# bbbranjan/scConsensus

Measured on AMD Instinct MI355X. Metric: end-to-end DE+distance cell-pairs/sec at config B (26k PBMC shape), higher is better.
Workload: dtype f64

## Files before the change

scconsensus_amd/csrc/scc_de.cpp:

```cpp
#include "scc_internal.hpp"

#include <array>
#include <cstring>
#include <memory>
#include <thread>

using namespace scc_rt;

enum { DE_FULL = 0, DE_SHARD = 1, DE_FINISH = 2, DE_SHARD_REC = 3, DE_FINISH_REC = 4 };

extern "C" {
int scc_rec_blocks(long long cells);
hipError_t scc_launch_rec_count(const uint8_t* flags, int G, int P, int glo, int ghi, int all, uint32_t* cnt,
                                hipStream_t st);
hipError_t scc_launch_rec_pack(const uint8_t* flags, int G, int P, int glo, int ghi, int all, const long long* off,
                               const double* p, const double* lfc, const double* pct1, const double* pct2,
                               const long long* u2, const long long* t, scc_de_record* out, hipStream_t st);
hipError_t scc_launch_rec_scatter(const scc_de_record* rec, long long n, int G, int P, double* p, double* lfc,
                                  double* pct1, double* pct2, long long* u2, long long* t, uint8_t* flags, int* err,
                                  int plo, int phi, hipStream_t st);
}

struct RecIO {
    void* out = nullptr;
// ... 9 lines not shown

extern "C" void scc_rank_split_diag(hipStream_t st, int ngenes);

enum IngestRoute {
    INGEST_NONE = 0,
    INGEST_FULL = 1,
    INGEST_LEAN = 2,
    INGEST_MIRROR = 3,
};

struct DePlan {
    const scc_dataset* ds;
    const scc_de_params* prm;
    void* shard;
    const RecIO* rio;
    int stage;
    bool shard_stage, finish_stage;
    bool pairs_only;
    int G, N, K, P, glo, ghi;
    int64_t GK, nnz1;
    size_t PG;
    bool fast, norank, all_pairs;
    bool markers;
    int test;
    std::vector<int> nclu;
    int nkept, nc, nc_kept, ns, gt, ntile, nwaves;
    size_t o_ccp0, o_cccode, o_sccc0, o_clcc, o_nclu, o_code8, tab_n;
    int ntp_max, cap_s, cap_m, wave_target, bucket_cap, item_cap, bucket_target;
    size_t acc_n;
    bool resplit, stamps;
    int fat_cap;
    IngestRoute route;
    bool try_mirror;
    double log_thr;
};

struct DeBuffers {
    int *d_tab, *d_nodg, *d_splitg, *d_counts, *d_err, *d_tested, *d_union, *d_nu, *d_genebk;
    const int *d_perm, *d_ccp0, *d_cccode, *d_sccc0, *d_clcc, *d_nclu;
    const signed char* d_code8;
    uint32_t *d_cnt, *d_cntpos, *d_cntneg, *d_gix, *d_gwin, *d_cscr;
    long long *d_gstart, *d_scan, *d_rowoff, *d_bnd;
    unsigned long long *d_keys, *d_keys2, *d_acc, *d_gkmin, *d_first;
    unsigned long long *accS, *accE, *accX, *accF;
    uint8_t *d_gcode, *d_gsc, *d_codes2, *d_flags;
    ScRankItem *d_items, *d_sbk;
    unsigned int* d_hbg;
    dd *d_wexp, *d_gexp;
    dd* d_sume;
    double *d_mx, *d_me, *d_vx, *d_mpos, *d_m2pos, *d_minpos, *d_maxpos;
    double *d_p, *d_lfc, *d_pct1, *d_pct2;
    long long *d_u2, *d_t;
    uint32_t* gene_tp;
    int* gene_nt;
    char* tp_scr;
    ScRankItem *fatbk, *fat2;
    int4 *rsseg, *fatg;
    unsigned long long* st_buf;
    uint32_t* d_rc;
    long long *d_roff, *d_rscr;
    int* d_row_gene;
    double *d_row_p, *d_row_q, *d_row_lfc, *d_row_pct1, *d_row_pct2;
    long long *d_row_u2, *d_row_t;
    uint8_t* d_row_flags;
    double* d_slow_q;
    uint8_t* d_slow_de;
// ... 399 lines not shown
    if (!ds->m_gptr) return SCC_OK;
    pl->route = INGEST_MIRROR;
    if (int rc = ensure_vorder(c, pl, B)) return rc;
    if (ds->d_tbnd) {
        hipFree(ds->d_tbnd);
        ds->d_tbnd = nullptr;
    }
    return SCC_OK;
}

static long long* gene_starts(const DePlan& pl, const DeBuffers& B)
{
    const bool whole = pl.glo == 0 && pl.ghi == pl.G;
    return pl.route == INGEST_MIRROR && whole && pl.nkept == pl.N ? pl.ds->m_gptr : B.d_gstart;
}

static int ingest_mirror(scc_ctx* c, const DePlan& pl, const DeBuffers& B)
{
    const scc_dataset* ds = pl.ds;
    const int G = pl.G, N = pl.N, K = pl.K, glo = pl.glo, ghi = pl.ghi, nc = pl.nc;
    hipStream_t s0 = c->s0;
    Scope sc(c, "ingest", s0);
    HIPCHK(c, scc_launch_de_clear(B.d_err, B.d_counts, pl.norank ? nullptr : B.d_acc, (long long)pl.acc_n, B.d_first,
                                  (int)G, glo, ghi, s0));
    HIPCHK(c, hipMemcpyAsync(B.d_nodg, ds->d_nodg, sizeof(int) * N, hipMemcpyDeviceToDevice, s0));
    const bool whole = glo == 0 && ghi == G;
    long long* gstart_run = gene_starts(pl, B);
    if (gstart_run == B.d_gstart) {
        uint32_t* d_total = B.d_cnt + (size_t)nc * G;
        if (!whole) HIPCHK(c, hipMemsetAsync(d_total, 0, sizeof(uint32_t) * G, s0));
        HIPCHK(c, scc_launch_mirror_total(ds->m_gptr, ds->m_cell, B.d_code8, glo, ghi, d_total, s0));
        HIPCHK(c, scc_launch_scan(d_total, G, B.d_gstart, B.d_scan, B.d_gstart + G, s0));
    }
    HIPCHK(c, scc_launch_mirror_regroup(ds->m_gptr, ds->m_cell, ds->m_key, B.d_code8, whole ? ds->m_order : nullptr,
                                        glo, ghi, K, G, B.d_clcc, gstart_run, B.d_cnt, B.d_keys, s0));
    return SCC_OK;
}

static int ingest_transpose(scc_ctx* c, const DePlan& pl, const DeBuffers& B)
{
    const scc_dataset* ds = pl.ds;
    const int G = pl.G, N = pl.N, glo = pl.glo, ghi = pl.ghi, nc = pl.nc, ntile = pl.ntile;
    const bool fast = pl.fast, lean = pl.route == INGEST_LEAN;
    const bool hist_rng = lean && (glo > 0 || ghi < G);
    const bool hist_ro = lean && !hist_rng;
    hipStream_t s0 = c->s0;
    Scope sc(c, "ingest", s0);
    HIPCHK(c, scc_launch_de_clear(B.d_err, B.d_counts, pl.norank ? nullptr : B.d_acc, (long long)pl.acc_n, B.d_first,
                                  (int)G, glo, ghi, s0));
    if (lean && !ds->d_tbnd) {
        const size_t tb_bytes = sizeof(long long) * (size_t)N * (ntile + 1);
        size_t mfree = 0, mtot = 0;
        const bool room = hipMemGetInfo(&mfree, &mtot) == hipSuccess && tb_bytes <= mfree / 4;
        (void)hipGetLastError();
        if (!room || hipMalloc((void**)&ds->d_tbnd, tb_bytes) != hipSuccess) {
            (void)hipGetLastError();
            ds->d_tbnd = nullptr;
        } else {
            HIPCHK(c, scc_launch_tile_bounds(ds->d_indptr, ds->d_rows, N, pl.gt, ntile, ds->d_tbnd, s0));
        }
    }
    const long long* tbnd = lean ? ds->d_tbnd : nullptr;
    if ((hist_ro || (hist_rng && ds->no_zeros)) && tbnd && env_int("SCC_COUNT_RO", 1) != 0)
        HIPCHK(c, scc_launch_ingest_count_ro(ds->d_indptr, ds->d_rows, G, B.d_perm, B.d_ccp0, B.d_cccode, nc,
                                             hist_rng ? glo : 0, hist_rng ? ghi : G, tbnd, B.d_cnt, s0));
    else
        HIPCHK(c, scc_launch_ingest_hist(ds->d_indptr, ds->d_rows, ds->d_vals, ds->d_dense, G, B.d_perm, B.d_ccp0,
                                         B.d_cccode, nc, ntile, B.d_cnt, B.d_bnd, B.d_nodg, B.d_wexp, fast ? 0 : 1, glo,
                                         ghi, hist_rng ? 1 : (hist_ro ? 2 : 0), tbnd, B.d_err, s0));
    if (lean) HIPCHK(c, hipMemcpyAsync(B.d_nodg, ds->d_nodg, sizeof(int) * N, hipMemcpyDeviceToDevice, s0));
    int cg0 = 0, cg1 = G;
    if (hist_rng) {
        scc_ingest_count_range(G, glo, ghi, &cg0, &cg1);
        HIPCHK(c, hipMemsetAsync(B.d_cnt + (size_t)nc * G, 0, sizeof(uint32_t) * G, s0));
    }
    HIPCHK(c, scc_launch_ingest_colscan(B.d_cnt, nc, pl.nc_kept, G, cg0, cg1, B.d_cscr, s0));
    const uint32_t* d_total = B.d_cnt + (size_t)nc * G;
    HIPCHK(c, scc_launch_scan(d_total, G, B.d_gstart, B.d_scan, B.d_gstart + G, s0));
    HIPCHK(c, scc_launch_ingest_scatter(ds->d_indptr, ds->d_rows, ds->d_vals, ds->d_dense, G, B.d_perm, B.d_ccp0,
                                        B.d_sccc0, pl.ns, B.d_cnt, B.d_gstart, B.d_bnd, tbnd, ntile, glo, ghi, B.d_keys,
                                        s0));
    if (!fast) HIPCHK(c, scc_launch_reduce_dd(B.d_wexp, pl.nwaves, B.d_gexp, s0));
    return SCC_OK;
}

static int gene_stats(scc_ctx* c, const DePlan& pl, const DeBuffers& B)
{
    Scope sc(c, "gene_stats", c->s0);
    ScStatsLaunch S{};
    S.gstart = gene_starts(pl, B);
    S.keys = B.d_keys;
    S.G = pl.G, S.K = pl.K, S.glo = pl.glo, S.gn = pl.ghi - pl.glo;
    S.mode = pl.prm->mode, S.test = pl.test;
    S.n_clu = B.d_nclu, S.coff = B.d_cnt, S.cl_cc = B.d_clcc;
    S.mean_x = B.d_mx, S.mean_e = B.d_me, S.cnt_pos = B.d_cntpos, S.cnt_neg = B.d_cntneg;
    S.var_x = B.d_vx;
    S.mean_pos = B.d_mpos, S.m2_pos = B.d_m2pos, S.min_pos = B.d_minpos, S.max_pos = B.d_maxpos;
    S.sum_e = B.d_sume;
    HIPCHK(c, scc_launch_gene_stats(&S, c->s0));
    return SCC_OK;
}

static int slow_threshold(scc_ctx* c, const DePlan& pl, const DeBuffers& B, double* log_thr)
{
    double gx[2];
    HIPCHK(c, hipMemcpyAsync(gx, B.d_gexp, sizeof(double) * 2, hipMemcpyDeviceToHost, c->s0));
    HIPCHK(c, hipStreamSynchronize(c->s0));
    const double tot = (double)pl.G * (double)pl.N;
    double q = gx[0] / tot;
    double r = std::fma(-q, tot, gx[0]) + gx[1];
    const double mean = q + r / tot;
    *log_thr = std::log(pl.prm->mean_scaling_factor * mean);
    return SCC_OK;
}

static ScTestLaunch test_launch(const scc_ctx* c, const DePlan& pl, const DeBuffers& B)
{
    ScTestLaunch T{};
    T.K = pl.K, T.G = pl.G, T.P = pl.P, T.glo = pl.glo, T.ghi = pl.ghi;
    T.mode = pl.prm->mode, T.test = pl.test, T.all_pairs = pl.all_pairs ? 1 : 0;
    T.min_pct = pl.prm->min_per_cent, T.lfc_thr = pl.prm->log_fc_thrs, T.log_thr = pl.log_thr;
// ... 24 lines not shown
    L.rw_mfma16 = env_int("SCC_RANK_MFMA16", -1);
    L.cross_wave = env_int("SCC_CROSS_WAVE", 0);
    L.bucket_cap = pl.bucket_cap, L.sbuckets = B.d_sbk, L.hbg = B.d_hbg;
    L.gene_bk = B.d_genebk, L.gkmin = B.d_gkmin;
    L.ntp_max = pl.ntp_max, L.item_cap = pl.item_cap, L.items = B.d_items;
    L.counts = B.d_counts, L.split_genes = B.d_splitg;
    L.keys2 = B.d_keys2, L.codes2 = B.d_codes2;
    L.gix = B.d_gix, L.gwin = B.d_gwin, L.gcode = B.d_gcode, L.gsc = B.d_gsc;
    L.nnz = pl.nnz1;
    L.accS = B.accS, L.accE = B.accE, L.accX = B.accX, L.accF = B.accF;
    L.gene_tp = B.gene_tp, L.gene_nt = B.gene_nt;
    if (scc_rank_tables_global(pl.ntp_max, K)) {
        L.tp_global = 1;
        L.tp_scr_stride = scc_rank_tables_stride(pl.ntp_max, K);
        L.tp_scr = B.tp_scr;
    }
    if (pl.resplit) {
        L.fat_cap = L.fat2_cap = pl.fat_cap;
        L.fatbk = B.fatbk, L.rsseg = B.rsseg, L.fatg = B.fatg, L.fat2 = B.fat2;
    }
    return L;
}

static int rank_log(scc_ctx* c, hipStream_t s0, const int* d_counts);

static bool rank_vorder_route(const scc_ctx* c, const DePlan& pl)
{
    const scc_dataset* ds = pl.ds;
    return ds->m_vcell && ds->m_vbk && ds->m_gptr && pl.route == INGEST_MIRROR && pl.fast && !pl.norank &&
           !pl.markers && !pl.shard_stage && pl.glo == 0 && pl.ghi == pl.G && c->peers.empty() &&
           ds->m_vnbk <= pl.bucket_cap && !pl.stamps && env_int("SCC_RANK_VORDER", 1) != 0;
}

static int rank_stage_vorder(scc_ctx* c, const DePlan& pl, const DeBuffers& B, ScRankLaunch& L)
{
    int rc;
    hipStream_t s0 = c->s0;
    const scc_dataset* ds = pl.ds;
    L.vcell = ds->m_vcell, L.vbk_ptr = ds->m_vbk_ptr, L.vbk = ds->m_vbk, L.vgptr = ds->m_gptr;
    L.code8 = B.d_code8;
    L.fatbk = nullptr;
    const int ncu = c->n_cu > 0 ? c->n_cu : 256;
    HIPCHK(c, scc_launch_rank_classify(&L, s0));
    HIPCHK(c, scc_launch_rank_vorder_list(&L, std::max(1, std::min((pl.G + 7) / 8, 1 << 20)), s0));
    if (L.dbg == 7) scc_rank_mfma_stamps(s0, 0);
    const int rw_side = (pl.K > 16 && env_int("SCC_RW_STREAMS", 1) != 0 && L.dbg != 7) ? 2 : 0;
    HIPCHK(c, scc_launch_rank_waves(&L, 8 * ncu, s0, c->sw, rw_side, c->ev_wfork, c->ev_wj));
    if (L.dbg == 7) scc_rank_mfma_stamps(s0, 1);
    HIPCHK(c, scc_launch_rank_cross(&L, 4 * ncu, s0));
    if (env_int("SCC_RANK_LOG", 0) && (rc = rank_log(c, s0, B.d_counts))) return rc;
    g_rank_last_route = 2;
    return SCC_OK;
}

static hipError_t read_counts(const int* d_counts, hipStream_t s0, int* h)
{
    int t[SCC_NCOUNTS * SCC_CNT_STRIDE];
    hipError_t e = hipMemcpyAsync(t, d_counts, sizeof(t), hipMemcpyDeviceToHost, s0);
    if (e == hipSuccess) e = hipStreamSynchronize(s0);
    for (int i = 0; i < SCC_NCOUNTS; ++i) h[i] = t[i * SCC_CNT_STRIDE];
    return e;
}

static int rank_stamps_begin(scc_ctx* c, hipStream_t s0, unsigned long long* st_buf, int item_cap, ScRankLaunch& L)
{
    HIPCHK(c, hipMemsetAsync(st_buf, 0, sizeof(unsigned long long) * 3 * item_cap * 8, s0));
// ... 40 lines not shown
}

static int rank_stamps_report(scc_ctx* c, hipStream_t s0, const unsigned long long* st_buf, int item_cap,
                              const int* d_counts)
{
    std::vector<unsigned long long> h((size_t)3 * item_cap * 8);
    int cnts[SCC_NCOUNTS];
    HIPCHK(c, hipMemcpyAsync(h.data(), st_buf, h.size() * 8, hipMemcpyDeviceToHost, s0));
    HIPCHK(c, read_counts(d_counts, s0, cnts));
    const char* ph[] = {"setup", "sort", "fixup+codes", "partition", "pairs", "ties"};
    fprintf(stderr, "[scc stamps] split genes %d\n", cnts[3]);
    for (int cls = 0; cls < 3; ++cls) {
        double acc[6] = {0, 0, 0, 0, 0, 0};
        int nb = 0;
        for (int b = 0; b < cnts[cls]; ++b) {
            const unsigned long long* t = &h[((size_t)cls * item_cap + b) * 8];
            if (!t[0] || !t[6]) continue;
            for (int q = 0; q < 6; ++q) acc[q] += (double)(t[q + 1] - t[q]);
            ++nb;
        }
        fprintf(stderr, "[scc stamps] rank class %d: %d items (%d full), mean cycles:", cls, cnts[cls], nb);
        for (int q = 0; q < 6; ++q) fprintf(stderr, " %s %.0f", ph[q], nb ? acc[q] / nb : 0.0);
        fprintf(stderr, "\n");
    }
    return SCC_OK;
}

static int rank_stage(scc_ctx* c, const DePlan& pl, const DeBuffers& B)
{
    int rc;
    hipStream_t s0 = c->s0, s1 = c->s1;
    Scope sc(c, "gene_rank", s0);
    ScRankLaunch L = rank_launch(pl, B);
    if (rank_vorder_route(c, pl)) return rank_stage_vorder(c, pl, B, L);
    if (pl.stamps && (rc = rank_stamps_begin(c, s0, B.st_buf, pl.item_cap, L))) return rc;
    HIPCHK(c, scc_launch_rank_classify(&L, s0));
    const int ncu = c->n_cu > 0 ? c->n_cu : 256;
    HIPCHK(c, scc_launch_rank_split(&L, 2 * ncu, s0));
    if (L.dbg >= 9 && (rc = rank_split_clocks(c, s0, B.d_counts))) return rc;
    if (pl.stamps) {
        if ((rc = rank_resplit_clocks(c, s0, L, B.st_buf, pl.item_cap, ncu))) return rc;
    } else {
        const int rw_mode = env_int("SCC_RW_STREAMS", 1);
        const int rs_side = (rw_mode >= 2 || (rw_mode != 0 && pl.ds->nnz > (64ll << 20))) ? 2 : 0;
        HIPCHK(c, scc_launch_rank_resplit(&L, 4 * ncu, s0, c->sw, rs_side, c->ev_wfork, c->ev_wj));
    }
    const bool items_serial = env_int("SCC_ITEMS_SERIAL", 0) != 0;
    hipStream_t si = items_serial ? s0 : s1;
    if (!items_serial) {
        HIPCHK(c, hipEventRecord(c->ev_fork, s0));
        HIPCHK(c, hipStreamWaitEvent(s1, c->ev_fork, 0));
    }
    if (L.dbg == 7) scc_rank_mfma_stamps(s0, 0);
    const int rw_side = (env_int("SCC_RW_STREAMS", 1) != 0 && L.dbg != 7) ? 2 : 0;
    const hipStream_t wsides[2] = {c->sw[0], si};
    HIPCHK(c, scc_launch_rank_waves(&L, 8 * ncu, s0, si != s0 ? wsides : c->sw, rw_side, c->ev_wfork, c->ev_wj));
    if (L.dbg == 7) scc_rank_mfma_stamps(s0, 1);
    HIPCHK(c, scc_launch_rank_items(&L, 1, 2 * ncu, si));
    HIPCHK(c, scc_launch_rank_items(&L, 0, 4 * ncu, si));
    HIPCHK(c, scc_launch_rank_items(&L, 2, ncu, si));
    if (!items_serial) {
        HIPCHK(c, hipEventRecord(c->ev_join, s1));
        HIPCHK(c, hipStreamWaitEvent(s0, c->ev_join, 0));
    }
    HIPCHK(c, scc_launch_rank_cross(&L, 4 * ncu, s0));
    HIPCHK(c, scc_launch_rank_cross_seg(&L, 4 * ncu, s0));
    if (env_int("SCC_RANK_LOG", 0) && (rc = rank_log(c, s0, B.d_counts))) return rc;
// ... 182 lines not shown
        r->n_rows = nrows;
    }
    r->d_nodg = B.d_nodg;
    r->d_row_gene = B.d_row_gene, r->d_row_p = B.d_row_p, r->d_row_q = B.d_row_q, r->d_row_lfc = B.d_row_lfc;
    r->d_row_pct1 = B.d_row_pct1, r->d_row_pct2 = B.d_row_pct2;
    r->d_row_u2 = B.d_row_u2, r->d_row_t = B.d_row_t, r->d_row_flags = B.d_row_flags;
    r->d_p = B.d_p, r->d_q = B.d_slow_q, r->d_lfc = B.d_lfc, r->d_u2 = B.d_u2, r->d_de = B.d_slow_de;
    return r;
}

static int de_run(scc_ctx* c, const scc_dataset* ds, const int32_t* code, int32_t K, const scc_de_params* prm,
                  int stage, int64_t glo64, int64_t ghi64, void* shard, scc_de_result** out,
                  const RecIO* rio = nullptr)
{
    int rc;
    if ((rc = de_check_args(c, ds, code, K, prm, stage, shard, out, rio))) return rc;
    scc_enter(c);
    DePlan pl{};
    if ((rc = de_plan(c, ds, code, K, prm, stage, glo64, ghi64, shard, rio, &pl))) return rc;
    DeBuffers B{};
    if ((rc = de_alloc(c, pl, &B))) return rc;
    if ((rc = ensure_wtab(c, exact_test_max_size(pl.nclu)))) return rc;
    hipStream_t s0 = c->s0;
    c->generation++;
    const int64_t sig[6] = {pl.G, pl.N, K, prm->mode, ds->nnz, (int64_t)(intptr_t)ds};
    if (pl.finish_stage) {
        if (!std::equal(sig, sig + 6, c->shard_sig))
            return fail(c, SCC_ERR_INVALID, "scc_de_finish: this context ran no scc_de_run_shard for these inputs");
        pl.log_thr = c->shard_log_thr;
        if ((rc = stage == DE_FINISH ? finish_load_dense(c, pl, B) : finish_scatter_records(c, pl, B))) return rc;
    } else {
        if ((rc = upload_tables(c, B))) return rc;
        if (pl.try_mirror && (rc = ensure_mirror(c, &pl, B))) return rc;
        g_ingest_last_path = pl.route;
        g_rank_last_route = 1;
        if ((rc = pl.route == INGEST_MIRROR ? ingest_mirror(c, pl, B) : ingest_transpose(c, pl, B))) return rc;
        if ((rc = gene_stats(c, pl, B))) return rc;
        if (!pl.fast && (rc = slow_threshold(c, pl, B, &pl.log_thr))) return rc;
        const ScTestLaunch T = test_launch(c, pl, B);
        {
            Scope sc(c, "pair_filter", s0);
            HIPCHK(c, scc_launch_pair_filter(&T, s0));
        }
        if (!pl.norank && (rc = rank_stage(c, pl, B))) return rc;
        {
            Scope sc(c, "pair_test", s0);
            HIPCHK(c, scc_launch_pair_test(&T, s0));
        }
    }
    if (pl.shard_stage) {
        if ((rc = stage == DE_SHARD ? shard_pack(c, pl, B) : shard_records(c, pl, B))) return rc;
        std::copy(sig, sig + 6, c->shard_sig);
        c->shard_log_thr = pl.log_thr;
        HIPCHK(c, hipStreamSynchronize(s0));
        int e = 0;
        HIPCHK(c, hipMemcpy(&e, B.d_err, sizeof(int), hipMemcpyDeviceToHost));
        if ((rc = de_error(c, e, AT_SHARD))) return rc;
        return note_validated(c, pl, B, e);
    }
    if ((rc = pair_select(c, pl, B)) || pl.pairs_only) return rc;
    if ((rc = stage_pack(c, pl, B))) return rc;
    const int n_union = c->h_stage[0], err_bits = c->h_stage[1];
    if ((rc = de_error(c, err_bits, AT_FULL))) return rc;
    if ((rc = note_validated(c, pl, B, err_bits))) return rc;
    if (n_union < 0 || n_union > pl.G) return fail(c, SCC_ERR_HIP, "union size out of range");
    *out = build_result(c, pl, B, n_union);
    return de_error(c, err_bits, AT_RESULT);
}
// ... 46 lines not shown
    return SCC_OK;
}

extern "C" int scc_de_markers(scc_ctx* c, const scc_dataset* ds, const int32_t* code, int32_t K,
                              const scc_markers_params* mp, scc_de_result** out)
{
    if (!c || !ds || !code || !mp || !out) return fail(c, SCC_ERR_INVALID, "scc_de_markers: null argument");
    *out = nullptr;
    if (ds->ctx != c) return fail(c, SCC_ERR_INVALID, "dataset belongs to another context");
    if (mp->test == SCC_TEST_T || mp->test == SCC_TEST_BIMOD)
        return fail(c, SCC_ERR_UNSUPPORTED, "scc_de_markers: SCC_TEST_WILCOX only");
    if (mp->test != SCC_TEST_WILCOX) return fail(c, SCC_ERR_INVALID, "scc_de_markers: bad test");
    if (K < 2) return fail(c, SCC_ERR_INVALID, "need at least two clusters");
    if (K > kMaxK) return fail(c, SCC_ERR_UNSUPPORTED, "scc_de_markers: K > 128 clusters");
    for (int32_t v : mp->reserved)
        if (v != 0) return fail(c, SCC_ERR_INVALID, "scc_de_markers: reserved fields must be zero");
    scc_de_params dp{};
    dp.mode = SCC_DE_FAST, dp.top_n = mp->top_n, dp.q_val_thrs = mp->q_val_thrs, dp.log_fc_thrs = mp->log_fc_thrs;
    dp.min_per_cent = mp->min_per_cent, dp.fc_thrs = 1.5, dp.mean_scaling_factor = 5.0;
    dp.test_all = mp->test_all ? 1 : 0, dp.test = SCC_TEST_WILCOX;
    int rc;
    scc_enter(c);
    DePlan pl{};
    if ((rc = markers_plan(c, ds, code, K, &dp, &pl))) return rc;
    DeBuffers B{};
    if ((rc = de_alloc(c, pl, &B))) return rc;
    if ((rc = ensure_wtab(c, markers_exact_size(pl.nclu)))) return rc;
    hipStream_t s0 = c->s0;
    c->generation++;
    if ((rc = upload_tables(c, B))) return rc;
    if (pl.try_mirror && (rc = ensure_mirror(c, &pl, B))) return rc;
    g_ingest_last_path = pl.route;
    g_rank_last_route = 1;
    if ((rc = pl.route == INGEST_MIRROR ? ingest_mirror(c, pl, B) : ingest_transpose(c, pl, B))) return rc;
    if ((rc = gene_stats(c, pl, B))) return rc;
    const ScRestTestLaunch T = rest_launch(c, pl, B, mp->only_pos ? 1 : 0);
    {
        Scope sc(c, "rest_filter", s0);
        HIPCHK(c, scc_launch_rest_filter(&T, s0));
    }
    if ((rc = rank_rest_stage(c, pl, B))) return rc;
    {
        Scope sc(c, "rest_test", s0);
        HIPCHK(c, scc_launch_rest_test(&T, s0));
    }
    if ((rc = pair_select(c, pl, B))) return rc;
    if ((rc = stage_pack(c, pl, B))) return rc;
    const int n_union = c->h_stage[0], err_bits = c->h_stage[1];
    if ((rc = de_error(c, err_bits, AT_FULL))) return rc;
    if ((rc = note_validated(c, pl, B, err_bits))) return rc;
    if (n_union < 0 || n_union > pl.G) return fail(c, SCC_ERR_HIP, "union size out of range");
    scc_de_result* r = build_result(c, pl, B, n_union);
    r->d_t = B.d_t;
    *out = r;
    return de_error(c, err_bits, AT_RESULT);
}

static int gene_blocks(scc_ctx* c, const scc_dataset* ds, int D, std::vector<int64_t>& cut)
{
    const int64_t G = ds->G;
    cut.assign(D + 1, 0);
    cut[D] = G;
    if (!ds->dense && ds->gene_w.empty() && ds->nnz > 0) {
        unsigned int* d_h = nullptr;
        int rc = ws(c, "row_hist", (size_t)G, &d_h);
        if (rc) return rc;
// ... 525 lines not shown
```

scconsensus_amd/csrc/scc_ingest.hip:

```cpp
#include "scc_common.hpp"
#include <algorithm>
#include "scc_kernels.hpp"

#define ING_T 256
#define IH_T (64 * SCC_ING_HIST_WAVES)

template <bool DENSE>
__device__ inline void cell_range(const i64* indptr, int c, int G, i64& b, i64& e)
{
    if (DENSE) {
        b = (i64)c * G;
        e = b + G;
    } else {
        b = indptr[c];
        e = indptr[c + 1];
    }
}

__device__ inline i64 wave_lower_bound(const int* __restrict__ rows, i64 lo, i64 hi, int v)
{
    const int lane = threadIdx.x & 63;
    while (hi - lo > 64) {
        const i64 step = (hi - lo + 63) / 64;
        const i64 k = lo + (i64)lane * step;
// ... 913 lines not shown
        }
        __syncthreads();
#pragma unroll
        for (int u = 0; u < MR_PER; ++u)
            if (aa[u] >= 0) {
                const u32 r = (u32)wc16[(wv * MR_PER + u) * SCC_MAX_K + aa[u]] + rk[u];
                const u32 slot = cst[aa[u]] + r;
                if (slot < (u32)MR_CH) {
                    skey[slot] = kk[u];
                    sdst[slot] = dbase[aa[u]] + r;
                }
            }
        __syncthreads();
        const int nk = (int)cst[K];
        for (int i0 = tid; i0 < nk; i0 += 4 * MR_T) {
            u64 kq[4];
            u32 dq[4];
#pragma unroll
            for (int q = 0; q < 4; ++q) {
                const int i = min(i0 + q * MR_T, nk - 1);
                kq[q] = skey[i];
                dq[q] = sdst[i];
            }
#pragma unroll
            for (int q = 0; q < 4; ++q)
                if (i0 + q * MR_T < nk) keys[gs + dq[q]] = kq[q];
        }
        if (c0 + MR_CH >= n) {
            if (tid <= K) cnt[(size_t)cl_cc[tid] * G + g] = coff[tid];
        }
    }
}

__global__ void __launch_bounds__(256) k_mir_segtab(const u32* __restrict__ cnt, int nch, int G, int nseg,
                                                    u32* __restrict__ seg)
{
    const int g = blockIdx.x * 256 + threadIdx.x;
    if (g >= G) return;
    for (int s = blockIdx.y; s <= nseg; s += gridDim.y)
        seg[(size_t)g * (nseg + 1) + s] = cnt[(size_t)min(s * (SCC_MIRROR_SEG / MR_BC), nch) * G + g];
}
static_assert(SCC_MIRROR_SEG % MR_BC == 0, "a cell segment is whole build chunks");

extern "C" hipError_t scc_launch_mirror_build(const i64* indptr, const int* rows, const double* vals, i64 nnz, int N,
                                              int G, u32* cnt, u32* colscan_scratch, i64* scan_scratch, i64* gptr,
                                              u32* mcell, u64* mkey, u32* mseg, hipStream_t st)
{
    const int nch = (N + MR_BC - 1) / MR_BC;
    hipError_t e = hipMemsetAsync(cnt, 0, sizeof(u32) * (size_t)nch * G, st);
    if (e != hipSuccess) return e;
    e = hipMemsetAsync(mcell, 0, sizeof(u32) * (size_t)std::max<i64>(1, nnz), st);
    if (e != hipSuccess) return e;
    hipLaunchKernelGGL(k_mir_bcount,dim3((nch + 3) / 4), dim3(256), 0, st, indptr, rows, vals, N, G, cnt);
    e = scc_launch_ingest_colscan(cnt, nch, nch, G, 0, G, colscan_scratch, st);
    if (e != hipSuccess) return e;
    e = scc_launch_scan(cnt + (size_t)nch * G, G, gptr, scan_scratch, gptr + G, st);
    if (e != hipSuccess) return e;
    if (mseg) {
        const int nseg = (N + SCC_MIRROR_SEG - 1) / SCC_MIRROR_SEG;
        hipLaunchKernelGGL(k_mir_segtab, dim3((G + 255) / 256, std::min(nseg + 1, 1024)), dim3(256), 0, st, cnt, nch,
                           G, nseg, mseg);
    }
    hipLaunchKernelGGL(k_mir_fill, dim3((nch + 3) / 4), dim3(256), 0, st, indptr, rows, vals, N, G, cnt, gptr, mcell,
                       mkey);
    return hipGetLastError();
}
// ... 22 lines not shown
```

scconsensus_amd/csrc/scc_kernels.hpp:

```cpp
#pragma once
#include <hip/hip_runtime.h>
#include <stdint.h>
#include <stddef.h>

#ifndef SCC_DE_FAST
#define SCC_DE_FAST 0
#define SCC_DE_SLOW 1
#endif
#ifndef SCC_TEST_T
#define SCC_TEST_WILCOX 0
#define SCC_TEST_T 1
#endif
#ifndef SCC_TEST_BIMOD
#define SCC_TEST_BIMOD 2
#endif

#define SCC_ING_HIST_WAVES 16

struct dd;

#define SCC_NCOUNTS 16
#define SCC_CNT_STRIDE 32

struct ScStatsLaunch {
// ... 190 lines not shown
                                  hipStream_t st);
int scc_ingest_colscan_scratch(int nc, int G);
hipError_t scc_launch_ingest_colscan(uint32_t* cnt, int nc, int nc_kept, int G, int g0, int g1, uint32_t* scratch,
                                     hipStream_t st);
void scc_ingest_count_range(int G, int glo, int ghi, int* g0, int* g1);
hipError_t scc_launch_ingest_scatter(const long long* indptr, const int* rows, const double* vals,
                                     const double* dense, int G, const int* perm, const int* cc_p0, const int* sc_cc0,
                                     int ns, const uint32_t* cnt, const long long* gstart, const long long* bnd,
                                     const long long* tbnd, int ntile, int glo, int ghi, unsigned long long* keys,
                                     hipStream_t st);
hipError_t scc_launch_ingest_count_ro(const long long* indptr, const int* rows, int G, const int* perm,
                                      const int* cc_p0, const int* cc_code, int nc, int glo, int ghi,
                                      const long long* tbnd, uint32_t* cnt, hipStream_t st);
hipError_t scc_launch_scan(const uint32_t* in, long long n, long long* out, long long* bsum_scratch,
                           long long* total, hipStream_t st);
int scc_scan_scratch_blocks(long long n);
#define SCC_MIRROR_SEG 128
hipError_t scc_launch_mirror_build(const long long* indptr, const int* rows, const double* vals, long long nnz, int N,
                                   int G, uint32_t* cnt, uint32_t* colscan_scratch, long long* scan_scratch,
                                   long long* gptr, uint32_t* mcell, unsigned long long* mkey, uint32_t* mseg,
                                   hipStream_t st);
hipError_t scc_launch_gather_mirror(const long long* gptr, const uint32_t* mcell, const unsigned long long* mkey,
                                    const uint32_t* mseg, int N, int Npad, const int* genes, int nu, int ld,
                                    double* Xc, hipStream_t st);
hipError_t scc_launch_center_mirror(const long long* gptr, const uint32_t* mcell, const unsigned long long* mkey,
                                    const uint32_t* mseg, double* Xc, int N, int nu, int ld, const int* genes,
                                    dd* part, int nchunk, double* mean, int apply, hipStream_t st);
hipError_t scc_launch_mirror_total(const long long* gptr, const uint32_t* mcell, const signed char* code, int glo,
                                   int ghi, uint32_t* total, hipStream_t st);
hipError_t scc_launch_mirror_regroup(const long long* gptr, const uint32_t* mcell, const unsigned long long* mkey,
                                     const signed char* code, const int* order, int glo, int ghi, int K, int G,
                                     const int* cl_cc, const long long* gstart, uint32_t* cnt,
                                     unsigned long long* keys, hipStream_t st);
hipError_t scc_launch_vorder_build(const long long* gptr, int G, const uint32_t* mcell, const unsigned long long* mkey,
                                   uint32_t* vcell, uint32_t* vbk_ptr, uint32_t** vbk_out, long long* nbk_out,
                                   uint32_t* cnt, long long* bptr, long long* scan_scratch, size_t vbk_max_bytes,
                                   unsigned long long* ks_lent, long long ks_n, void* tmp_lent, size_t tmp_lent_bytes,
                                   hipStream_t st);
struct ScCsrPlan {
    long long G, N, nnz;
    int SB, NS;
    int T;
    int CG, NG;
    size_t off_bnd, off_rs, off_tt, off_ts, off_off, off_gm, off_gb, off_scan, off_meta, off_ival, bytes;
};
int scc_csr_plan(long long G, long long N, long long nnz, ScCsrPlan* P);
hipError_t scc_launch_csr_check(const ScCsrPlan* P, const long long* indptr, const int* cols, void* scratch,
                                int* err, hipStream_t st);
hipError_t scc_launch_csr_to_csc(const ScCsrPlan* P, const long long* indptr, const int* cols, const double* vals,
                                 void* scratch, long long* csc_indptr, int* csc_rows, double* csc_vals,
                                 hipStream_t st);
hipError_t scc_launch_reduce_dd(const dd* parts, int n, dd* out, hipStream_t st);

hipError_t scc_launch_gene_stats(const ScStatsLaunch* L, hipStream_t st);
hipError_t scc_launch_rank_classify(const ScRankLaunch* L, hipStream_t st);
size_t scc_rank_item_lds(int cls, int cap, int ntp_max, int K);
int scc_rank_item_cap(int cls, int want, int ntp_max, int K, int lim);
size_t scc_rank_split_lds(int K);
int scc_rank_tables_global(int ntp_max, int K);
size_t scc_rank_tables_stride(int ntp_max, int K);
hipError_t scc_launch_rank_split(const ScRankLaunch* L, int grid, hipStream_t st);
hipError_t scc_launch_rank_items(const ScRankLaunch* L, int cls, int grid, hipStream_t st);
hipError_t scc_launch_rank_vorder_list(const ScRankLaunch* L, int grid, hipStream_t st);
hipError_t scc_launch_rank_waves(const ScRankLaunch* L, int grid, hipStream_t st, const hipStream_t* side = nullptr,
                                 int nside = 0, hipEvent_t fork = nullptr, const hipEvent_t* join = nullptr);
void scc_rank_mfma_stamps(hipStream_t st, int print);
// ... 89 lines not shown
```

scconsensus_amd/csrc/scc_rank.hip:

```cpp
#include "scc_common.hpp"
#include "scc_kernels.hpp"

#include <algorithm>
#include <cstddef>
#include <cstdio>
#include <vector>
#include <type_traits>

__device__ inline u64 f_tie(u64 c) { return c * c * c - c; }

__device__ inline u32 lanes_below(u64 m)
{
    return __builtin_amdgcn_mbcnt_hi((u32)(m >> 32), __builtin_amdgcn_mbcnt_lo((u32)m, 0u));
}

__device__ inline u64 shfl_xor_u64(u64 v, int m)
{
    const u32 lo = __shfl_xor((u32)v, m, 64), hi = __shfl_xor((u32)(v >> 32), m, 64);
    return ((u64)hi << 32) | lo;
}

__device__ inline void pair_decode(int p, int K, int& a, int& b)
{
    a = 0;
    int rem = p;
    while (rem >= K - 1 - a) {
        rem -= K - 1 - a;
        ++a;
    }
    b = a + 1 + rem;
}

template <int BITS>
__device__ inline u64 match_bits(u32 d, u64 act)
{
    u64 peers = act;
#pragma unroll
    for (int b = 0; b < BITS; ++b) {
        const bool bit = (d >> b) & 1u;
        const u64 bb = __ballot(bit);
        peers &= bit ? bb : ~bb;
    }
    return peers;
}

#define ST_T 256
#define ST_W (ST_T / 64)
#ifndef ST_U
#define ST_U 4
#endif

struct StatItem {
    double sx_hi, sx_lo, se_hi, se_lo;
    u32 pos, neg;
};

struct StatMinMax {
    double mn, mx;
};

template <bool MAX>
__device__ inline double f64_wave_ext_dpp(double x)
{
    auto ext = [](double a, double b) { return MAX ? fmax(a, b) : fmin(a, b); };
    x = ext(x, scc_xor_lane_f64<32>(x));
    x = ext(x, scc_xor_lane_f64<16>(x));
    x = ext(x, scc_xor_lane_f64<8>(x));
    x = ext(x, scc_xor_lane_f64<4>(x));
    x = ext(x, scc_xor_lane_f64<2>(x));
    return ext(x, scc_xor_lane_f64<1>(x));
}

#define ST_NITEM (SCC_MAX_K + ST_W + 4)
static_assert(sizeof(int) * (SCC_MAX_K + 1) + (sizeof(StatItem) + sizeof(StatMinMax)) * ST_NITEM <= 16 * 1024,
              "k_gene_stats: static LDS (off[], item[], mm[]) beyond 16 KiB a workgroup");

template <bool EXPM1, bool SUMX, bool VAR, bool POS = false, bool SUME = false>
__global__ void __launch_bounds__(ST_T) k_gene_stats(ScStatsLaunch A)
{
    __shared__ int off[SCC_MAX_K + 1];
// ... 3017 lines not shown
```

Measured before the change: 144.5 billion.

## Compute Wilcoxon gene stats directly from mirror, skipping regroup pass

Adds a k_mir_stats kernel that reads the gene-major mirror (cells, keys) and produces mean expm1, positive and negative counts per cluster directly. When the vorder rank route is taken with a Wilcoxon test and K is small enough, it drops the mirror regroup that writes clustered keys plus the separate gene_stats kernel. The kernel does a per-chunk ballot-based counting sort by cluster code in LDS and uses double-double reductions paced to match k_gene_stats' wave partitioning. The aim is to cut a full keys write and re-read. It adds a complex kernel with LDS pressure, and correctness depends on the later stages not needing d_keys on this route.

```diff
diff --git a/scconsensus_amd/csrc/scc_de.cpp b/scconsensus_amd/csrc/scc_de.cpp
--- a/scconsensus_amd/csrc/scc_de.cpp
+++ b/scconsensus_amd/csrc/scc_de.cpp
@@ -65,6 +65,7 @@
     int fat_cap;
     IngestRoute route;
     bool try_mirror;
+    bool vorder, stats_mirror;
     double log_thr;
 };
 
@@ -530,8 +531,10 @@
         HIPCHK(c, scc_launch_mirror_total(ds->m_gptr, ds->m_cell, B.d_code8, glo, ghi, d_total, s0));
         HIPCHK(c, scc_launch_scan(d_total, G, B.d_gstart, B.d_scan, B.d_gstart + G, s0));
     }
-    HIPCHK(c, scc_launch_mirror_regroup(ds->m_gptr, ds->m_cell, ds->m_key, B.d_code8, whole ? ds->m_order : nullptr,
-                                        glo, ghi, K, G, B.d_clcc, gstart_run, B.d_cnt, B.d_keys, s0));
+    if (!pl.stats_mirror)
+        HIPCHK(c, scc_launch_mirror_regroup(ds->m_gptr, ds->m_cell, ds->m_key, B.d_code8,
+                                            whole ? ds->m_order : nullptr, glo, ghi, K, G, B.d_clcc, gstart_run,
+                                            B.d_cnt, B.d_keys, s0));
     return SCC_OK;
 }
 
@@ -585,6 +588,12 @@
 static int gene_stats(scc_ctx* c, const DePlan& pl, const DeBuffers& B)
 {
     Scope sc(c, "gene_stats", c->s0);
+    if (pl.stats_mirror) {
+        const scc_dataset* ds = pl.ds;
+        HIPCHK(c, scc_launch_mirror_stats(ds->m_gptr, ds->m_cell, ds->m_key, B.d_code8, ds->m_order, pl.G, pl.K,
+                                          gene_starts(pl, B), B.d_nclu, B.d_me, B.d_cntpos, B.d_cntneg, c->s0));
+        return SCC_OK;
+    }
     ScStatsLaunch S{};
     S.gstart = gene_starts(pl, B);
     S.keys = B.d_keys;
@@ -675,6 +684,12 @@
            ds->m_vnbk <= pl.bucket_cap && !pl.stamps && env_int("SCC_RANK_VORDER", 1) != 0;
 }
 
+static bool stats_mirror_route(const DePlan& pl)
+{
+    return pl.vorder && pl.test == SCC_TEST_WILCOX && pl.ds->m_order && pl.K <= scc_mirror_stats_max_k() &&
+           env_int("SCC_STATS_MIRROR", 1) != 0;
+}
+
 static int rank_stage_vorder(scc_ctx* c, const DePlan& pl, const DeBuffers& B, ScRankLaunch& L)
 {
     int rc;
@@ -781,7 +796,7 @@
     hipStream_t s0 = c->s0, s1 = c->s1;
     Scope sc(c, "gene_rank", s0);
     ScRankLaunch L = rank_launch(pl, B);
-    if (rank_vorder_route(c, pl)) return rank_stage_vorder(c, pl, B, L);
+    if (pl.vorder) return rank_stage_vorder(c, pl, B, L);
     if (pl.stamps && (rc = rank_stamps_begin(c, s0, B.st_buf, pl.item_cap, L))) return rc;
     HIPCHK(c, scc_launch_rank_classify(&L, s0));
     const int ncu = c->n_cu > 0 ? c->n_cu : 256;
@@ -1030,8 +1045,11 @@
     } else {
         if ((rc = upload_tables(c, B))) return rc;
         if (pl.try_mirror && (rc = ensure_mirror(c, &pl, B))) return rc;
+        pl.vorder = rank_vorder_route(c, pl);
+        pl.stats_mirror = stats_mirror_route(pl);
         g_ingest_last_path = pl.route;
         g_rank_last_route = 1;
+        g_mirror_last_uses = (g_mirror_last_uses & ~1) | (pl.stats_mirror ? 1 : 0);
         if ((rc = pl.route == INGEST_MIRROR ? ingest_mirror(c, pl, B) : ingest_transpose(c, pl, B))) return rc;
         if ((rc = gene_stats(c, pl, B))) return rc;
         if (!pl.fast && (rc = slow_threshold(c, pl, B, &pl.log_thr))) return rc;
@@ -1144,6 +1162,7 @@
     if (pl.try_mirror && (rc = ensure_mirror(c, &pl, B))) return rc;
     g_ingest_last_path = pl.route;
     g_rank_last_route = 1;
+    g_mirror_last_uses &= ~1;
     if ((rc = pl.route == INGEST_MIRROR ? ingest_mirror(c, pl, B) : ingest_transpose(c, pl, B))) return rc;
     if ((rc = gene_stats(c, pl, B))) return rc;
     const ScRestTestLaunch T = rest_launch(c, pl, B, mp->only_pos ? 1 : 0);
diff --git a/scconsensus_amd/csrc/scc_ingest.hip b/scconsensus_amd/csrc/scc_ingest.hip
--- a/scconsensus_amd/csrc/scc_ingest.hip
+++ b/scconsensus_amd/csrc/scc_ingest.hip
@@ -969,6 +969,237 @@
     }
 }
 
+#define MS_T 256
+#define MS_CH 1024
+#define MS_PER (MS_CH / MS_T)
+#define MS_NS (MS_CH / 64)
+#define MS_TPR (MS_T / MS_NS)
+#define MS_W (MS_T / 64)
+#define MS_KREG (4 * MS_W)
+#define MS_KLDS 36
+static_assert(MS_KREG <= 16 && MS_KLDS <= 64, "k_mir_stats: 4 and 6 code bits in the match");
+
+template <int NB>
+__device__ inline u64 ms_match(int a, bool act)
+{
+    u64 m = __ballot(act);
+#pragma unroll
+    for (int b = 0; b < NB; ++b) {
+        const bool bit = (a >> b) & 1;
+        const u64 bb = __ballot(bit);
+        m &= bit ? bb : ~bb;
+    }
+    return m;
+}
+
+__device__ inline dd ms_wave_sum4(const dd (&x)[4], int lane)
+{
+    const dd s0 = dd_add(x[0], dd_xor_lane<32>(x[0])), s1 = dd_add(x[1], dd_xor_lane<32>(x[1]));
+    const dd s2 = dd_add(x[2], dd_xor_lane<32>(x[2])), s3 = dd_add(x[3], dd_xor_lane<32>(x[3]));
+    const bool up = lane & 32;
+    dd m01{up ? s1.hi : s0.hi, up ? s1.lo : s0.lo}, m23{up ? s3.hi : s2.hi, up ? s3.lo : s2.lo};
+    m01 = dd_add(m01, dd_xor_lane<16>(m01));
+    m23 = dd_add(m23, dd_xor_lane<16>(m23));
+    const bool odd = lane & 16;
+    dd m{odd ? m23.hi : m01.hi, odd ? m23.lo : m01.lo};
+    m = dd_add(m, dd_xor_lane<8>(m));
+    m = dd_add(m, dd_xor_lane<4>(m));
+    m = dd_add(m, dd_xor_lane<2>(m));
+    return dd_add(m, dd_xor_lane<1>(m));
+}
+
+__device__ inline void ms_walk(const double* sval, u32 c0s, u32 cn, u32 rb, u32 Lp, int lane, dd& acc, dd* tot,
+                               u32& nxt)
+{
+    for (u32 r0 = rb & ~63u; r0 < rb + cn; r0 += 64u) {
+        if (r0 == nxt) {
+            const dd t = dd_add(*tot, dd_wave_sum_dpp(acc));
+            *tot = t;
+            acc = dd{0.0, 0.0};
+            nxt += Lp;
+        }
+        const u32 rr = r0 + (u32)lane;
+        if (rr >= rb && rr < rb + cn) acc = dd_add_d(acc, sval[c0s + (rr - rb)]);
+    }
+}
+
+template <bool REG>
+__global__ void __launch_bounds__(MS_T, 6) k_mir_stats(const i64* __restrict__ gptr, const u32* __restrict__ mcell,
+                                                    const u64* __restrict__ mkey,
+                                                    const signed char* __restrict__ code,
+                                                    const int* __restrict__ order, int K, int G,
+                                                    const i64* __restrict__ gstart, const int* __restrict__ n_clu,
+                                                    double* __restrict__ mean_e, u32* __restrict__ cnt_pos,
+                                                    u32* __restrict__ cnt_neg)
+{
+    __shared__ double sval[MS_CH];
+    __shared__ u32 wc[MS_NS][SCC_MAX_K / 2];
+    __shared__ u32 cst[SCC_MAX_K + 1];
+    __shared__ u32 rbase[SCC_MAX_K];
+    __shared__ u32 cneg[SCC_MAX_K];
+    __shared__ u32 snxt[SCC_MAX_K];
+    __shared__ dd stot[SCC_MAX_K];
+    extern __shared__ dd ms_acc[];
+    const int tid = threadIdx.x, lane = tid & 63, wv = scc_wave_id();
+    const int g = order[blockIdx.x];
+    const i64 b = gptr[g];
+    const int n = (int)(gptr[g + 1] - b);
+    const int nk = (int)(gstart[g + 1] - gstart[g]);
+    const u32 Lp = (u32)max(64, (((nk + SCC_STATS_WAVES - 1) / SCC_STATS_WAVES) + 63) & ~63);
+    const u64 below = (1ull << lane) - 1ull;
+    if (tid < SCC_MAX_K) {
+        cneg[tid] = 0u;
+        snxt[tid] = Lp;
+        stot[tid] = dd{0.0, 0.0};
+    }
+    dd acc[MS_KREG / MS_W];
+    u32 nxt[MS_KREG / MS_W];
+#pragma unroll
+    for (int q = 0; q < MS_KREG / MS_W; ++q) acc[q] = dd{0.0, 0.0}, nxt[q] = Lp;
+    if (!REG)
+        for (int i = tid; i < K * 64; i += MS_T) ms_acc[i] = dd{0.0, 0.0};
+    unsigned short* const wc16 = (unsigned short*)&wc[0][0];
+    const int kw = (K + 1) >> 1;
+    u32 run0 = 0u, run1 = 0u;
+    static_assert(MS_T / 64 * MS_PER == MS_NS && MS_NS % 8 == 0, "k_mir_stats: a wc row per MS_TPR threads");
+    for (int c0 = 0; c0 < n; c0 += MS_CH) {
+        const int len = min(MS_CH, n - c0);
+        for (int q = tid % MS_TPR; q < kw; q += MS_TPR) wc[tid / MS_TPR][q] = 0u;
+        u32 cl[MS_PER];
+        u64 kk[MS_PER];
+#pragma unroll
+        for (int u = 0; u < MS_PER; ++u) {
+            const int ic = min(wv * (64 * MS_PER) + u * 64 + lane, len - 1);
+            cl[u] = mcell[b + c0 + ic];
+            kk[u] = mkey[b + c0 + ic];
+        }
+        int aa[MS_PER];
+        u32 rk[MS_PER];
+        double ev[MS_PER];
+        u32 sgn = 0u;
+#pragma unroll
+        for (int u = 0; u < MS_PER; ++u) {
+            const int i = wv * (64 * MS_PER) + u * 64 + lane;
+            const int a = (int)code[cl[u]];
+            const double x = scc_val_of(kk[u]);
+            aa[u] = i < len ? a : -1;
+            sgn |= (u32)(~kk[u] >> 63) << u;
+            ev[u] = expm1(x);
+        }
+        __syncthreads();
+#pragma unroll
+        for (int u = 0; u < MS_PER; ++u) {
+            const bool act = aa[u] >= 0;
+            const u64 m = ms_match<REG ? 4 : 6>(aa[u], act);
+            const u64 mn = __ballot(act && ((sgn >> u) & 1u));
+            rk[u] = (u32)__popcll(m & below);
+            if (act && rk[u] == 0u) wc16[(wv * MS_PER + u) * SCC_MAX_K + aa[u]] = (unsigned short)__popcll(m);
+            if (mn != 0ull && act && rk[u] == 0u) {
+                const u32 nn = (u32)__popcll(m & mn);
+                if (nn) atomicAdd(&cneg[aa[u]], nn);
+            }
+        }
+        __syncthreads();
+        if (wv == 0) {
+            u32 sum = 0u;
+            if (lane < kw) {
+                for (int s0 = 0; s0 < MS_NS; s0 += 8) {
+                    u32 x[8];
+#pragma unroll
+                    for (int s = 0; s < 8; ++s) x[s] = wc[s0 + s][lane];
+#pragma unroll
+                    for (int s = 0; s < 8; ++s) {
+                        wc[s0 + s][lane] = sum;
+                        sum += x[s];
+                    }
+                }
+            }
+            const u32 v0 = sum & 0xffffu, v1 = sum >> 16;
+            u32 inc = v0 + v1;
+            for (int o = 1; o < 64; o <<= 1) {
+                const u32 y = __shfl_up(inc, o, 64);
+                if (lane >= o) inc += y;
+            }
+            cst[2 * lane] = inc - v0 - v1;
+            cst[2 * lane + 1] = inc - v1;
+            if (lane == 63) cst[SCC_MAX_K] = inc;
+            rbase[2 * lane] = run0;
+            rbase[2 * lane + 1] = run1;
+            run0 += v0;
+            run1 += v1;
+        }
+        __syncthreads();
+#pragma unroll
+        for (int u = 0; u < MS_PER; ++u)
+            if (aa[u] >= 0) {
+                const u32 slot = cst[aa[u]] + (u32)wc16[(wv * MS_PER + u) * SCC_MAX_K + aa[u]] + rk[u];
+                if (slot < (u32)MS_CH) sval[slot] = ev[u];
+            }
+        __syncthreads();
+        if (REG) {
+#pragma unroll
+            for (int q = 0; q < MS_KREG / MS_W; ++q) {
+                const int a = q * MS_W + wv;
+                if (a < K) {
+                    const u32 c0s = (u32)__builtin_amdgcn_readfirstlane((int)cst[a]);
+                    const u32 cn = (u32)__builtin_amdgcn_readfirstlane((int)cst[a + 1]) - c0s;
+                    const u32 rb = (u32)__builtin_amdgcn_readfirstlane((int)rbase[a]);
+                    if (cn) ms_walk(sval, c0s, cn, rb, Lp, lane, acc[q], &stot[a], nxt[q]);
+                }
+            }
+        } else {
+            for (int a = wv; a < K; a += MS_W) {
+                const u32 c0s = (u32)__builtin_amdgcn_readfirstlane((int)cst[a]);
+                const u32 cn = (u32)__builtin_amdgcn_readfirstlane((int)cst[a + 1]) - c0s;
+                const u32 rb = (u32)__builtin_amdgcn_readfirstlane((int)rbase[a]);
+                if (cn) {
+                    dd s = ms_acc[a * 64 + lane];
+                    u32 nx = (u32)__builtin_amdgcn_readfirstlane((int)snxt[a]);
+                    ms_walk(sval, c0s, cn, rb, Lp, lane, s, &stot[a], nx);
+                    ms_acc[a * 64 + lane] = s;
+                    snxt[a] = nx;
+                }
+            }
+        }
+    }
+    __syncthreads();
+    for (int a0 = wv; a0 < K; a0 += MS_KREG) {
+        dd x[MS_KREG / MS_W];
+#pragma unroll
+        for (int q = 0; q < MS_KREG / MS_W; ++q) {
+            const int a = a0 + q * MS_W;
+            x[q] = REG ? acc[q] : (a < K ? ms_acc[a * 64 + lane] : dd{0.0, 0.0});
+        }
+        const dd m = ms_wave_sum4(x, lane);
+        const int a = a0 + MS_W * (((lane >> 5) & 1) | ((lane >> 3) & 2));
+        if (a < K && (lane & 15) == 0) {
+            const dd t = dd_add(stot[a], m);
+            const u32 all = n > 0 ? rbase[a] + cst[a + 1] - cst[a] : 0u;
+            mean_e[(size_t)a * G + g] = dd_div_n(t, (double)n_clu[a]);
+            cnt_pos[(size_t)a * G + g] = all - cneg[a];
+            cnt_neg[(size_t)a * G + g] = cneg[a];
+        }
+    }
+}
+
+extern "C" int scc_mirror_stats_max_k(void) { return MS_KLDS; }
+
+extern "C" hipError_t scc_launch_mirror_stats(const i64* gptr, const u32* mcell, const u64* mkey,
+                                              const signed char* code, const int* order, int G, int K,
+                                              const i64* gstart, const int* n_clu, double* mean_e, u32* cnt_pos,
+                                              u32* cnt_neg, hipStream_t st)
+{
+    if (G <= 0) return hipSuccess;
+    if (K < 1 || K > MS_KLDS) return hipErrorInvalidValue;
+    if (K <= MS_KREG)
+        hipLaunchKernelGGL((k_mir_stats<true>), dim3(G), dim3(MS_T), 0, st, gptr, mcell, mkey, code, order, K, G,
+                           gstart, n_clu, mean_e, cnt_pos, cnt_neg);
+    else
+        hipLaunchKernelGGL((k_mir_stats<false>), dim3(G), dim3(MS_T), sizeof(dd) * 64 * (size_t)K, st, gptr, mcell,
+                           mkey, code, order, K, G, gstart, n_clu, mean_e, cnt_pos, cnt_neg);
+    return hipGetLastError();
+}
+
 __global__ void __launch_bounds__(256) k_mir_segtab(const u32* __restrict__ cnt, int nch, int G, int nseg,
                                                     u32* __restrict__ seg)
 {
diff --git a/scconsensus_amd/csrc/scc_kernels.hpp b/scconsensus_amd/csrc/scc_kernels.hpp
--- a/scconsensus_amd/csrc/scc_kernels.hpp
+++ b/scconsensus_amd/csrc/scc_kernels.hpp
@@ -246,6 +246,12 @@
                                      const signed char* code, const int* order, int glo, int ghi, int K, int G,
                                      const int* cl_cc, const long long* gstart, uint32_t* cnt,
                                      unsigned long long* keys, hipStream_t st);
+#define SCC_STATS_WAVES 4
+int scc_mirror_stats_max_k(void);
+hipError_t scc_launch_mirror_stats(const long long* gptr, const uint32_t* mcell, const unsigned long long* mkey,
+                                   const signed char* code, const int* order, int G, int K, const long long* gstart,
+                                   const int* n_clu, double* mean_e, uint32_t* cnt_pos, uint32_t* cnt_neg,
+                                   hipStream_t st);
 hipError_t scc_launch_vorder_build(const long long* gptr, int G, const uint32_t* mcell, const unsigned long long* mkey,
                                    uint32_t* vcell, uint32_t* vbk_ptr, uint32_t** vbk_out, long long* nbk_out,
                                    uint32_t* cnt, long long* bptr, long long* scan_scratch, size_t vbk_max_bytes,
diff --git a/scconsensus_amd/csrc/scc_rank.hip b/scconsensus_amd/csrc/scc_rank.hip
--- a/scconsensus_amd/csrc/scc_rank.hip
+++ b/scconsensus_amd/csrc/scc_rank.hip
@@ -46,6 +46,7 @@
 
 #define ST_T 256
 #define ST_W (ST_T / 64)
+static_assert(ST_W == SCC_STATS_WAVES, "k_mir_stats (scc_ingest.hip) repeats k_gene_stats' pieces");
 #ifndef ST_U
 #define ST_U 4
 #endif
```

Result: faster. 157.6 billion (median of 6 runs) (+9.0%).
